# AWehenkel/UMNN

Measured on AMD Instinct MI355X. Metric: umnn_maf_log_density_evals_per_s, higher is better.
Workload: dtype f32 via f16x3-split MFMA (fp32 accumulate)

## Files before the change

### umnn_amd/csrc/cc_api.hip

```cpp
#include <atomic>
#include <cmath>
#include <cstring>
#include <mutex>
#include <unordered_map>
#include <vector>

#include "cc_host.h"

static thread_local char g_err[512] = "";
static thread_local const char* g_last_kernel = "";
static std::atomic<long long> g_launches{0};

int umnn_fail(int code, const char* msg) {
    snprintf(g_err, sizeof(g_err), "%s", msg);
    return code;
}

int umnn_check(hipError_t e, const char* what) {
    if (e == hipSuccess) return 0;
    snprintf(g_err, sizeof(g_err), "%s: %s", what, hipGetErrorString(e));
    return (int)e;
}

static std::atomic<const char*> g_last_of[3] = {{""}, {""}, {""}};
void umnn_note_launch(const char* kernel_name) {
    g_last_kernel = kernel_name;
    const int tag = !strncmp(kernel_name, "cc_bwd_dh", 9) || !strncmp(kernel_name, "cc_bwd_reduce", 13) ? UMNN_PROF_FINISH
                    : !strncmp(kernel_name, "cc_bwd", 6) ? UMNN_PROF_BACKWARD : UMNN_PROF_FORWARD;
    g_last_of[tag].store(kernel_name, std::memory_order_relaxed);
    g_launches.fetch_add(1, std::memory_order_relaxed);
}
static std::atomic<long long> g_made_launches{0};
static std::atomic<const char*> g_last_made{""};
void umnn_note_made_launch(const char* kernel_name) {
    g_last_made.store(kernel_name, std::memory_order_relaxed);
    g_made_launches.fetch_add(1, std::memory_order_relaxed);
}
extern "C" long long umnn_made_launch_count(void) { return g_made_launches.load(std::memory_order_relaxed); }
extern "C" const char* umnn_last_made_kernel_name(void) { return g_last_made.load(std::memory_order_relaxed); }
extern "C" const char* umnn_last_kernel_name_of(int tag) {
    return tag >= 0 && tag <= 2 ? g_last_of[tag].load(std::memory_order_relaxed) : "";
}

int umnn_num_cus() {
    static std::atomic<int> cus[64];
    int dev = 0;
    if (hipGetDevice(&dev) != hipSuccess || dev < 0 || dev >= 64) return 256;
    int v = cus[dev].load(std::memory_order_relaxed);
    if (!v) {
        hipDeviceProp_t prop;
        v = hipGetDeviceProperties(&prop, dev) == hipSuccess && prop.multiProcessorCount > 0 ? prop.multiProcessorCount : 256;
        cus[dev].store(v, std::memory_order_relaxed);
    }
    return v;
}

int umnn_ovf_slot(unsigned long long** flag, unsigned long long* gen) {
    static std::mutex mu;
    static unsigned long long* ring[64] = {nullptr};
    static std::atomic<unsigned long long> next{1};
    int dev = 0;
    if (int rc = umnn_check(hipGetDevice(&dev), "hipGetDevice")) return rc;
// ... 22 lines not shown
int umnn_allow_lds(const void* fn, size_t bytes) {
    struct Key { int dev; const void* fn; bool operator==(const Key& o) const { return dev == o.dev && fn == o.fn; } };
    struct Hash { size_t operator()(const Key& k) const { return std::hash<const void*>()(k.fn) ^ ((size_t)k.dev * 0x9e3779b97f4a7c15ull); } };
    static std::mutex mu;
    static std::unordered_map<Key, size_t, Hash> granted;
    int dev = 0;
    if (int rc = umnn_check(hipGetDevice(&dev), "hipGetDevice")) return rc;
    std::lock_guard<std::mutex> lk(mu);
    auto it = granted.find(Key{dev, fn});
    if (it != granted.end() && it->second >= bytes) return 0;
    if (int rc = umnn_check(hipFuncSetAttribute(fn, hipFuncAttributeMaxDynamicSharedMemorySize, (int)bytes),
                            "hipFuncSetAttribute(MaxDynamicSharedMemorySize)"))
        return rc;
    granted[Key{dev, fn}] = bytes;
    return 0;
}

static int env_int(const char* name, int dflt) { const char* e = getenv(name); return e && *e ? atoi(e) : dflt; }
static void load_env(UmnnOptions& o) {
    int fp = UMNN_PRECISION_F16X3, bp = UMNN_PRECISION_BF16X3;
    if (const char* ev = getenv("UMNN_FWD_PRECISION")) {
        if (!strcmp(ev, "fp32")) fp = UMNN_PRECISION_FP32;
        else if (!strcmp(ev, "bf16x6")) fp = UMNN_PRECISION_BF16X6;
        else if (!strcmp(ev, "bf16x3")) fp = UMNN_PRECISION_BF16X3;
    }
    if (const char* ev = getenv("UMNN_BWD_PRECISION")) bp = !strcmp(ev, "fp32") ? UMNN_PRECISION_FP32 : UMNN_PRECISION_BF16X3;
    o.fwd_precision = fp; o.bwd_precision = bp;
    int v = env_int("UMNN_FWD_P", -1); o.fwd_p = v == 1 || v == 2 ? v : -1;
    v = env_int("UMNN_FWD_NS", -1); o.fwd_ns = v == 1 || v == 2 || v == 4 ? v : -1;
    v = env_int("UMNN_FWD_TAIL", -1); o.fwd_tail = v < 0 ? -1 : (v != 0);
    v = env_int("UMNN_FWD_PIPE", 1); o.fwd_pipe = v >= 0 && v <= 2 ? v : 1;
    o.fwd_pad = env_int("UMNN_FWD_PAD", 1) != 0;
    v = env_int("UMNN_FWD_PAD_MIN", 1); o.fwd_pad_min = v >= 0 && v <= 127 ? v : 1;
    v = env_int("UMNN_BWD_NS", -1); o.bwd_ns = v >= 1 && v <= 32 ? v : -1;
    o.bwd_swp = env_int("UMNN_BWD_SWP", 1) != 0;
    o.bwd_ws = env_int("UMNN_BWD_WS", 1) != 0;
    v = env_int("UMNN_BWD_WS16", 1); o.bwd_ws16 = v >= 0 && v <= 2 ? v : 1;
    v = env_int("UMNN_FRONT_BWD2", 1); o.front_bwd2 = v >= 0 && v <= 2 ? v : 1;
}
UmnnOptions& umnn_options() {
    static UmnnOptions opts;
    static std::once_flag once;
    std::call_once(once, [] { load_env(opts); });
    return opts;
}
extern "C" int umnn_reload_env(void) { load_env(umnn_options()); return 0; }

static std::atomic<int>* option_slot(const char* name) {
    UmnnOptions& o = umnn_options();
    if (!name) return nullptr;
    if (!strcmp(name, "fwd_precision")) return &o.fwd_precision;
    if (!strcmp(name, "bwd_precision")) return &o.bwd_precision;
    if (!strcmp(name, "fwd_p")) return &o.fwd_p;
    if (!strcmp(name, "fwd_ns")) return &o.fwd_ns;
    if (!strcmp(name, "fwd_tail")) return &o.fwd_tail;
    if (!strcmp(name, "fwd_pipe")) return &o.fwd_pipe;
    if (!strcmp(name, "fwd_pad")) return &o.fwd_pad;
    if (!strcmp(name, "fwd_pad_min")) return &o.fwd_pad_min;
    if (!strcmp(name, "bwd_ns")) return &o.bwd_ns;
    if (!strcmp(name, "bwd_swp")) return &o.bwd_swp;
    if (!strcmp(name, "bwd_ws")) return &o.bwd_ws;
    if (!strcmp(name, "bwd_ws16")) return &o.bwd_ws16;
    if (!strcmp(name, "front_bwd2")) return &o.front_bwd2;
    return nullptr;
}
static bool option_value_ok(const char* name, int v) {
    if (!strcmp(name, "fwd_precision")) return v >= UMNN_PRECISION_FP32 && v <= UMNN_PRECISION_F16X3;
    if (!strcmp(name, "bwd_precision")) return v == UMNN_PRECISION_FP32 || v == UMNN_PRECISION_BF16X3;
    if (!strcmp(name, "fwd_p")) return v == -1 || v == 1 || v == 2;
    if (!strcmp(name, "fwd_ns")) return v == -1 || v == 1 || v == 2 || v == 4;
    if (!strcmp(name, "fwd_tail")) return v == -1 || v == 0 || v == 1;
    if (!strcmp(name, "fwd_pipe")) return v >= 0 && v <= 2;
    if (!strcmp(name, "fwd_pad")) return v == 0 || v == 1;
    if (!strcmp(name, "fwd_pad_min")) return v >= 0 && v <= 127;
    if (!strcmp(name, "bwd_ns")) return v == -1 || (v >= 1 && v <= 32);
    if (!strcmp(name, "bwd_swp")) return v == 0 || v == 1;
    if (!strcmp(name, "bwd_ws")) return v == 0 || v == 1;
    if (!strcmp(name, "bwd_ws16")) return v >= 0 && v <= 2;
    if (!strcmp(name, "front_bwd2")) return v >= 0 && v <= 2;
    return true;
}
extern "C" int umnn_set_option(const char* name, int value) {
    std::atomic<int>* s = option_slot(name);
    if (!s) return umnn_fail(UMNN_EINVAL, "umnn_set_option: unknown option name");
    if (!option_value_ok(name, value)) return umnn_fail(UMNN_EINVAL, "umnn_set_option: value out of range for this option");
    s->store(value, std::memory_order_relaxed);
    return 0;
}
extern "C" int umnn_get_option(const char* name, int* value) {
    std::atomic<int>* s = option_slot(name);
    if (!s || !value) return umnn_fail(UMNN_EINVAL, "umnn_get_option: unknown option name or null output");
    *value = s->load(std::memory_order_relaxed);
    return 0;
}
extern "C" int umnn_set_forward_precision(int mode) {
    if (mode < UMNN_PRECISION_FP32 || mode > UMNN_PRECISION_F16X3) return umnn_fail(UMNN_EINVAL, "unknown precision mode");
    umnn_options().fwd_precision = mode;
    return 0;
}
extern "C" int umnn_get_forward_precision(void) { return umnn_options().fwd_precision; }
extern "C" int umnn_set_backward_precision(int mode) {
    if (mode != UMNN_PRECISION_FP32 && mode != UMNN_PRECISION_BF16X3)
        return umnn_fail(UMNN_EINVAL, "backward precision must be UMNN_PRECISION_FP32 or UMNN_PRECISION_BF16X3");
    umnn_options().bwd_precision = mode;
    return 0;
}
extern "C" int umnn_get_backward_precision(void) { return umnn_options().bwd_precision; }
// ... 154 lines not shown
```

### umnn_amd/csrc/cc_common.h

```cpp
#pragma once
#include <hip/hip_runtime.h>

#include "../../include/umnn_cc.h"

typedef float f32x4 __attribute__((ext_vector_type(4)));

#define UMNN_WAVES_PER_BLOCK 4
#define UMNN_BLOCK (64 * UMNN_WAVES_PER_BLOCK)

struct MlpDev {
    const float* W[UMNN_MAX_LINEAR];
    const float* b[UMNN_MAX_LINEAR];
    int width[UMNN_MAX_LINEAR + 1];
    int n_linear;
    int t_out[UMNN_MAX_LINEAR];
    int ks_in[UMNN_MAX_LINEAR];
    int lds_off[UMNN_MAX_LINEAR];
    int t_mfma[UMNN_MAX_LINEAR];
    int tail_off;
    int n_tail;
    int hidden_act;
    int out_act;
};

__device__ __forceinline__ int feat_of(int t, int r, int g) { return 16 * t + 4 * r + g; }
__device__ __forceinline__ int fout_of(int t, int rho) { return 16 * t + 4 * (rho & 3) + (rho >> 2); }

__device__ __forceinline__ f32x4 mfma16(float a, float b, f32x4 c) {
    return __builtin_amdgcn_mfma_f32_16x16x4f32(a, b, c, 0, 0, 0);
}

__device__ __forceinline__ unsigned short f32_to_bf16_rn(float x) {
    const unsigned u = __float_as_uint(x);
    return (unsigned short)((u + 0x7fffu + ((u >> 16) & 1u)) >> 16);
}
__device__ __forceinline__ float io_ld(const float* p, long long i, int bf16) {
    return bf16 ? __uint_as_float((unsigned)reinterpret_cast<const unsigned short*>(p)[i] << 16) : p[i];
}
__device__ __forceinline__ void io_st(float* p, long long i, float v, int bf16) {
    if (bf16) reinterpret_cast<unsigned short*>(p)[i] = f32_to_bf16_rn(v);
    else p[i] = v;
}
struct IoView {
    const float* p;
    int bf16;
    __device__ __forceinline__ float operator[](long long i) const { return io_ld(p, i, bf16); }
    __device__ __forceinline__ IoView operator+(long long o) const {
        return IoView{bf16 ? reinterpret_cast<const float*>(reinterpret_cast<const unsigned short*>(p) + o) : p + o, bf16};
    }
};

template <int NT, int CH>
__device__ __forceinline__ void item_embedding_gemm(const IoView& hb, const float* __restrict__ W0, int H1, int E, int d, int g, int p,
                                                    f32x4 (&c)[NT]) {
    for (int se0 = 0; se0 < (E + 3) / 4; se0 += CH) {
        float hv[CH], A[CH][NT];
#pragma unroll
        for (int q = 0; q < CH; ++q) {
            const int e = 4 * (se0 + q) + g;
// ... 92 lines not shown
```

### umnn_amd/csrc/cc_forward_bf16.hip

```cpp
#ifndef UMNN_ASM_TIED
#define UMNN_ASM_TIED 1
#endif
#include "cc_fwd_plan.h"
using namespace UMNN_FWD_NS;
#ifdef UMNN_FWD_PIECE_F16
#define FWD_KNAME "cc_fwd_f16"
#define FWD_LAUNCH umnn_launch_forward_f16
#else
#define FWD_KNAME "cc_fwd_bf16"
#define FWD_LAUNCH umnn_launch_forward_bf16
#endif

typedef void (*fwd_bf16_kernel_t)(const FwdBf16Args);
struct Bf16Variant { int tmax, nparts, p, exact, nrl, pipe, wpb; fwd_bf16_kernel_t fn; const char* name; };
struct Bf16WideFirst { int t1, nrl, p; fwd_bf16_kernel_t fn; const char* name; };
#define BF16_WIDE_FIRST(T, NR, PP) { T, NR, PP, cc_fwd_bf16_kernel<T, 2, PP, true, NR, false, false, 4>, FWD_KNAME "<T1=" #T ",TREST=4,PARTS=2,P=" #PP ",EXACT=1,LIVE=" #NR ">" }
static const Bf16WideFirst kBf16WideFirst[] = { BF16_WIDE_FIRST(5, 13, 1), BF16_WIDE_FIRST(6, 13, 1), BF16_WIDE_FIRST(7, 13, 1), BF16_WIDE_FIRST(8, 13, 1),
                                                BF16_WIDE_FIRST(5, 0, 1), BF16_WIDE_FIRST(6, 0, 1), BF16_WIDE_FIRST(7, 0, 1), BF16_WIDE_FIRST(8, 0, 1) };
#define BF16_VARIANT(T, NP, PP, EX, NR) { T, NP, PP, EX, NR, 0, 4, cc_fwd_bf16_kernel<T, NP, PP, (EX) != 0, NR>, FWD_KNAME "<T=" #T ",PARTS=" #NP ",P=" #PP ",EXACT=" #EX ",LIVE=" #NR ">" }
#define BF16_PIPE_VARIANT(NP, PP, NR) { 4, NP, PP, 1, NR, 1, 4, cc_fwd_bf16_kernel<4, NP, PP, true, NR, true>, FWD_KNAME "<T=4,PARTS=" #NP ",P=" #PP ",EXACT=1,LIVE=" #NR ",PIPE>" }
#define BF16_VARIANT_W8(T, NR) { T, 2, 1, 1, NR, 0, 8, cc_fwd_bf16_kernel<T, 2, 1, true, NR, false, false, 0, 8>, FWD_KNAME "<T=" #T ",PARTS=2,P=1,EXACT=1,LIVE=" #NR ",WAVES=8>" }
static const Bf16Variant kBf16Variants[] = {
    BF16_PIPE_VARIANT(2, 2, 13), BF16_PIPE_VARIANT(2, 2, 0),
    BF16_VARIANT(4, 2, 1, 1, 13), BF16_VARIANT(4, 2, 2, 1, 13),
    BF16_VARIANT(4, 2, 1, 1, 0), BF16_VARIANT(4, 2, 2, 1, 0),
    BF16_VARIANT(2, 2, 1, 0, 0), BF16_VARIANT(2, 2, 2, 0, 0),
    BF16_VARIANT(4, 2, 1, 0, 0), BF16_VARIANT(4, 2, 2, 0, 0),
#ifndef UMNN_FWD_PIECE_F16
    BF16_VARIANT(4, 3, 1, 1, 13), BF16_VARIANT(4, 3, 2, 1, 13), BF16_VARIANT(4, 3, 1, 1, 0), BF16_VARIANT(4, 3, 2, 1, 0),
    BF16_VARIANT(2, 3, 1, 0, 0), BF16_VARIANT(2, 3, 2, 0, 0), BF16_VARIANT(4, 3, 1, 0, 0), BF16_VARIANT(4, 3, 2, 0, 0),
#endif
    BF16_VARIANT(7, 2, 1, 1, 26), BF16_VARIANT(7, 2, 1, 1, 0),
    BF16_VARIANT(5, 2, 1, 1, 0), BF16_VARIANT(6, 2, 1, 1, 0), BF16_VARIANT(8, 2, 1, 1, 0),
    BF16_VARIANT_W8(7, 26), BF16_VARIANT_W8(7, 0), BF16_VARIANT_W8(5, 0), BF16_VARIANT_W8(6, 0), BF16_VARIANT_W8(8, 0),
    BF16_VARIANT(8, 2, 1, 0, 0), BF16_VARIANT(8, 2, 2, 0, 0),
};

int umnn_launch_forward_p32(FwdArgs& a, const umnn_mlp* net, int nb_steps, hipStream_t stream);

struct FwdOvfPlan { int mode; unsigned long long* flag; unsigned long long gen; };
int umnn_ovf_slot(unsigned long long** flag, unsigned long long* gen);
#ifdef UMNN_FWD_PIECE_F16
int umnn_launch_forward_bf16(FwdArgs& a, const umnn_mlp* net, int nparts, int P, int ns, int nb_steps, hipStream_t stream,
                             const FwdOvfPlan* ovf);
#endif

static int launch_planned(fwd_bf16_kernel_t fn, const char* name, unsigned nblk, size_t lds_bytes, FwdBf16Args& args, FwdArgs& a,
                          const umnn_mlp* net, int P, int ns, int nb_steps, hipStream_t stream, const FwdOvfPlan* ovf, int block) {
    args.f.ovf_mode = ovf ? ovf->mode : 0;
    args.f.ovf_flag = ovf ? ovf->flag : nullptr;
    args.f.ovf_gen = ovf ? ovf->gen : 0;
#ifdef UMNN_FWD_PIECE_F16
    umnn_prof_begin(stream);
    hipLaunchKernelGGL(fn, dim3(nblk), dim3(block), lds_bytes, stream, args);
    const FwdOvfPlan second{2, ovf->flag, ovf->gen};
    int rc = umnn_check(hipGetLastError(), "cc_fwd_f16 launch");
    if (!rc) rc = umnn_launch_forward_bf16(a, net, 2, P, ns, nb_steps, stream, &second);
    if (rc == UMNN_EUNSUPPORTED) rc = umnn_fail(UMNN_EUNSUPPORTED, "cc_fwd_f16: the bf16 build has no kernel for the plan of the fp16 launch");
    umnn_prof_end(stream, umnn_cc_forward_flops_per_integral(net, nb_steps) * (double)a.NI);
    umnn_note_launch(name);
    return rc;
#else
    (void)P; (void)ns;
    if (!ovf) umnn_prof_begin(stream);
    hipLaunchKernelGGL(fn, dim3(nblk), dim3(block), lds_bytes, stream, args);
    if (!ovf) {
        umnn_prof_end(stream, umnn_cc_forward_flops_per_integral(net, nb_steps) * (double)a.NI);
        umnn_note_launch(name);
    }
    return umnn_check(hipGetLastError(), "cc_fwd_bf16 launch");
#endif
}

int FWD_LAUNCH(FwdArgs& a, const umnn_mlp* net, int nparts, int P, int ns, int nb_steps,
                             hipStream_t stream, const FwdOvfPlan* ovf) {
    const int L = a.m.n_linear - 1;
    const UmnnOptions& opt = umnn_options();
#ifdef UMNN_FWD_PIECE_F16
    FwdOvfPlan own{1, nullptr, 0};
    if (int rc = umnn_ovf_slot(&own.flag, &own.gen)) return rc;
    ovf = &own;
    const bool fb = false;
#else
    const bool fb = ovf != nullptr;
#endif
    const bool p_forced = opt.fwd_p > 0 || fb, ns_forced = opt.fwd_ns > 0 || fb;
    int tmax = 0;
    for (int l = 1; l <= L; ++l) tmax = a.m.t_out[l] > tmax ? a.m.t_out[l] : tmax;
    int wide = nparts == 2 ? fwd_uniform_wide(a.m, tmax) : 0;
    if (wide && (P == 1 || !p_forced)) P = 1; else wide = 0;
    if (wide && !ns_forced) {
        const long long tiles16 = (a.NI + 15) / 16, slots = (long long)umnn_num_cus() * 8;
        ns = tiles16 * 4 <= slots ? 4 : tiles16 * 2 <= slots ? 2 : 1;
        if (ns > nb_steps + 1) ns = 1;
    }
    FwdBf16Args args;
    args.f = a;
    FwdLayout lay;
    if (nparts == 2 && (P == 1 || !p_forced) && fwd_plan_wide_first(args, nparts, &lay)) {
        if (!ns_forced) {
            const long long tiles16 = (a.NI + 15) / 16, slots = (long long)umnn_num_cus() * 4 * 2;
            ns = tiles16 * 4 <= slots ? 4 : tiles16 * 2 <= slots ? 2 : 1;
            if (ns > nb_steps + 1) ns = 1;
        }
        const size_t lds_bytes = ((size_t)args.f.m.lds_off[L] + (ns > 1 ? UMNN_WAVES_PER_BLOCK * 3 * 16 : 0)) * sizeof(float);
        const Bf16WideFirst* pick = nullptr;
        for (const Bf16WideFirst& v : kBf16WideFirst) if (v.t1 == lay.T && v.nrl == lay.nrl && v.p == 1) pick = &v;
        if (pick && lds_bytes <= 160 * 1024) {
            if (int rc = umnn_allow_lds((const void*)pick->fn, lds_bytes)) return rc;
            args.f.ns = ns;
            args.f.ngroups = (unsigned)((a.NI + 16 * pick->p - 1) / (16 * pick->p));
            const unsigned gpb = UMNN_WAVES_PER_BLOCK / ns;
            const unsigned nblk = (args.f.ngroups + gpb - 1) / gpb;
            return launch_planned(pick->fn, pick->name, nblk, lds_bytes, args, a, net, pick->p, ns, nb_steps, stream, ovf, UMNN_BLOCK);
        }
        args.f = a;
    }
    if (a.z2_save) return UMNN_EUNSUPPORTED;
    lay = fwd_plan_images(args, nparts, tmax, wide, nparts == 2 && opt.fwd_pad, opt.fwd_pad_min);
    const int T = lay.T, exact = lay.exact, nrl = lay.nrl;
    const bool want_pipe = opt.fwd_pipe != 0 && L >= 2;
#ifndef UMNN_FWD_PIECE_F16
    if (opt.fwd_pipe == 2 && !fb && exact && T == 4 && nparts == 2 && nrl == 13) {
        const int rc = umnn_launch_forward_p32(a, net, nb_steps, stream);
        if (rc != UMNN_EUNSUPPORTED) return rc;
    }
#endif
    if (want_pipe && exact && T == 4 && nparts == 2 && !p_forced && !ns_forced &&
        (a.NI + 15) / 16 >= 2LL * umnn_num_cus() * 4) { P = 2; ns = 1; }
    int wpb = wide && exact && 2 * ((size_t)args.f.m.lds_off[L] * sizeof(float) + 1024) > 160 * 1024 ? 8 : UMNN_WAVES_PER_BLOCK;
    size_t lds_bytes = ((size_t)args.f.m.lds_off[L] + (ns > 1 ? wpb * 3 * P * 16 : 0)) * sizeof(float);
    if (lds_bytes > 160 * 1024 && wpb == 8) { wpb = UMNN_WAVES_PER_BLOCK; lds_bytes = ((size_t)args.f.m.lds_off[L] + (ns > 1 ? wpb * 3 * P * 16 : 0)) * sizeof(float); }
    if (lds_bytes > 160 * 1024) return UMNN_EUNSUPPORTED;
    const Bf16Variant* pick = nullptr;
    for (int ex = exact; ex >= 0 && !pick; --ex)
        for (int pass = 0; pass < 2 && !pick; ++pass)
            for (const Bf16Variant& v : kBf16Variants)
                if (v.tmax == T && v.nparts == nparts && v.p == P && v.exact == ex && (!v.pipe || want_pipe) && v.wpb == (ex ? wpb : 4) &&
                    (pass == 0 ? (ex && nrl && v.nrl == nrl) : v.nrl == 0)) { pick = &v; break; }
    if (!pick) return UMNN_EUNSUPPORTED;
    fwd_bf16_kernel_t kfn = pick->fn;
    const char* kname = pick->name;
    if (int rc = umnn_allow_lds((const void*)kfn, lds_bytes)) return rc;
    args.f.ns = ns;
    args.f.ngroups = (unsigned)((a.NI + 16 * P - 1) / (16 * P));
    const unsigned gpb = pick->wpb / ns;
    const unsigned nblk = (args.f.ngroups + gpb - 1) / gpb;
    return launch_planned(kfn, kname, nblk, lds_bytes, args, a, net, P, ns, nb_steps, stream, ovf, 64 * pick->wpb);
}
```

### umnn_amd/csrc/cc_fwd_bf16_kernel.h

```cpp
#pragma once
#include <type_traits>
#include <utility>
#include "cc_bf16.h"
#include "cc_fwd_shared.h"
#include "cc_host.h"

#ifdef UMNN_FWD_PIECE_F16
#define UMNN_FWD_NS fwd_f16
#else
#define UMNN_FWD_NS fwd_bf16
#endif
namespace UMNN_FWD_NS {
#ifdef UMNN_FWD_PIECE_F16
typedef _Float16 pc_x8 __attribute__((ext_vector_type(8)));
typedef _Float16 pc_x4 __attribute__((ext_vector_type(4)));
typedef _Float16 pc_x2 __attribute__((ext_vector_type(2)));
constexpr unsigned PC_MINUS_ONE = 0xBC00u;
constexpr bool PC_F16 = true;
__device__ __forceinline__ f32x4 pc_mfma(u32x4 a, u32x4 b, f32x4 c) {
    return __builtin_amdgcn_mfma_f32_16x16x32_f16(__builtin_bit_cast(pc_x8, a), __builtin_bit_cast(pc_x8, b), c, 0, 0, 0);
}
__device__ __forceinline__ f32x4 pc_mfma_k16(u32x2 a, u32x2 b, f32x4 c) {
    return __builtin_amdgcn_mfma_f32_16x16x16f16(__builtin_bit_cast(pc_x4, a), __builtin_bit_cast(pc_x4, b), c, 0, 0, 0);
}
// ... 20 lines not shown
}
#ifdef UMNN_FWD_PIECE_F16
__device__ __forceinline__ unsigned pc_lo_pair(float x0, float x1, unsigned hi) {
    unsigned lo = __float_as_uint(x0);
    asm("v_fma_mixlo_f16 %0, %1, -1.0, %0 op_sel_hi:[1,0,0]" : "+v"(lo) : "v"(hi));
    asm("v_fma_mixhi_f16 %0, %1, -1.0, %2 op_sel:[1,0,0] op_sel_hi:[1,0,0]" : "+v"(lo) : "v"(hi), "v"(x1));
    return lo;
}
template <int I>
__device__ __forceinline__ void pc_sub_halves(f32x4& v, unsigned bits) {
    float x0 = v[I], x1 = v[I + 1];
    asm("v_fma_mix_f32 %0, %1, -1.0, %0 op_sel_hi:[1,0,0]" : "+v"(x0) : "v"(bits));
    asm("v_fma_mix_f32 %0, %1, -1.0, %0 op_sel:[1,0,0] op_sel_hi:[1,0,0]" : "+v"(x1) : "v"(bits));
    v[I] = x0; v[I + 1] = x1;
}
#endif
template <int NPARTS>
__device__ __forceinline__ void pc_split_pair(float x0, float x1, unsigned (&out)[NPARTS]) {
#ifdef UMNN_FWD_PIECE_F16
    if constexpr (NPARTS == 2) {
        out[0] = pc_cvt_pk(x0, x1);
        out[1] = pc_lo_pair(x0, x1, out[0]);
        return;
    }
#endif
#pragma unroll
    for (int k = 0; k < NPARTS; ++k) {
        const unsigned bits = pc_cvt_pk(x0, x1);
        out[k] = bits;
        if (k + 1 < NPARTS) { x0 -= pc_lo_f32(bits); x1 -= pc_hi_f32(bits); }
    }
}

template <int NPARTS, int MERGE_FROM = 0>
__device__ __forceinline__ void stage_bf16_images(const MlpDev& m, const int* ks32, const int* off16, const int* half_in,
                                                  unsigned short* lds16, int tid, int nthreads) {
    const int L = m.n_linear - 1;
    for (int l = 1; l < L; ++l) {
        const int Hin = m.width[l], Hout = m.width[l + 1];
        const int ks = ks32[l], to = m.t_out[l + 1];
        const float* __restrict__ W = m.W[l];
        const float* __restrict__ b = m.b[l];
        unsigned short* img = lds16 + off16[l];
        auto wv = [&](int fo, int fi) {
            float v = 0.f;
            if (fo < Hout) {
                if (fi < Hin) v = W[fo * Hin + fi];
                else if (fi == Hin) v = b[fo];
            } else if (fo == Hout && fi == Hin) {
                v = 1.f;
            }
            return v;
        };
        auto split8 = [&](const float (&v)[8], unsigned (&pk)[NPARTS][4]) {
#pragma unroll
            for (int e = 0; e < 4; ++e) {
                unsigned q[NPARTS];
                pc_split_pair<NPARTS>(v[2 * e], v[2 * e + 1], q);
#pragma unroll
                for (int part = 0; part < NPARTS; ++part) pk[part][e] = q[part];
            }
        };
        const int total = to * ks * 64;
        for (int idx = tid; idx < total; idx += nthreads) {
            const int ln = idx & 63, ts = idx >> 6;
            const int s = ts % ks, t = ts / ks;
// ... 25 lines not shown
                unsigned q0[NPARTS], q1[NPARTS];
                pc_split_pair<NPARTS>(wv(fo, feat_of(2 * ks, 0, g)), wv(fo, feat_of(2 * ks, 1, g)), q0);
                pc_split_pair<NPARTS>(wv(fo, feat_of(2 * ks, 2, g)), wv(fo, feat_of(2 * ks, 3, g)), q1);
#pragma unroll
                for (int part = 0; part < NPARTS; ++part)
                    *reinterpret_cast<u32x2*>(himg + (t * NPARTS + part) * 256 + ln * 4) = u32x2{q0[part], q1[part]};
            }
        }
    }
}

struct Bf16Plan {
    int ks32[UMNN_MAX_LINEAR];
    int off16[UMNN_MAX_LINEAR];
    int half_in[UMNN_MAX_LINEAR];
    int scratch_off_floats;
};

struct SolveArgs {
    long long t_stride = 0, x_stride = 0;
    const float* scale_row = nullptr;
    const float* off_row = nullptr;
    int off_h0 = 0;
    int* status = nullptr;
    float lo = 0.f, hi = 0.f, tol = 0.f;
    int block = 0;
};
constexpr int SOLVE_CLAMPED = 1 << 16, SOLVE_CAPPED = 1 << 17, SOLVE_NONFINITE = 1 << 18;

struct FwdBf16Args {
    FwdArgs f;
    Bf16Plan pl;
    SolveArgs sv;
};

template <int... I, class F>
__device__ __forceinline__ void static_for(std::integer_sequence<int, I...>, F&& f) {
    (f(std::integral_constant<int, I>{}), ...);
}
template <int TMAX, int NPARTS, int P, bool EXACT, int NRL, bool PIPE = false, int INV = 0, int TREST = 0, int WPB = UMNN_WAVES_PER_BLOCK>
__global__ __launch_bounds__(64 * WPB) void cc_fwd_bf16_kernel(const FwdBf16Args args) {
    static_assert(TREST == 0 || (EXACT && !PIPE && TREST < TMAX && (TREST & 1) == 0), "wide-first-layer variants: exact, plain loop");
    static_assert(!INV || (P == 1 && !PIPE), "inversion variants: plain loop, one tile per wave");
    constexpr int KSM = TMAX / 2;
    constexpr int NLIVE = (NRL > 0 && TREST == 0) ? NRL : 4 * TMAX;
    constexpr int NREST = TREST > 0 ? (NRL > 0 ? NRL : 4 * TREST) : NLIVE;
    constexpr bool MERGE = EXACT && TMAX == 4 && NRL == 13 && NPARTS == 2 && TREST == 0;
    constexpr bool MERGE_REST = EXACT && TREST == 4 && NRL == 13 && NPARTS == 2;
    extern __shared__ __attribute__((aligned(16))) float lds[];
    const FwdArgs& a = args.f;
    const MlpDev& m = a.m;
    const int tid = threadIdx.x, lane = tid & 63;
    const int wid = __builtin_amdgcn_readfirstlane(tid >> 6);
    const int g = lane >> 4, p = lane & 15;
    const int L = m.n_linear - 1;
    const int H1 = m.width[1], HL = m.width[L];
    const int E = a.E, d = a.d, n = a.n;
    const float slope = m.hidden_act == UMNN_ACT_RELU ? 0.f : 0.01f;
    unsigned short* lds16 = reinterpret_cast<unsigned short*>(lds);
    if (a.ovf_mode == 2 && *a.ovf_flag < a.ovf_gen) return;

    stage_bf16_images<NPARTS, MERGE ? 1 : MERGE_REST ? 2 : 0>(m, args.pl.ks32, args.pl.off16, args.pl.half_in, lds16, tid, 64 * WPB);
    __syncthreads();

    const int ns = a.ns;
    const int sub = wid / ns, part = wid % ns;
    const unsigned gpb = WPB / ns;
    const unsigned grp = xcd_remap(blockIdx.x, gridDim.x) * gpb + sub;
    bool live = grp < a.ngroups;
    if (a.ovf_mode == 2 && live) {
        if constexpr (INV == 2) {
            long long q = (long long)grp * 16 + p;
            if (q >= a.NI) q = a.NI - 1;
            const float v = a.inv_x[q * args.sv.x_stride + a.inv_j];
            live = __any(v != v);
        } else if constexpr (INV) { const float v = a.inv_x[(long long)grp * d + a.inv_j]; live = v != v; }
        else live = fwd_group_marked<P>(a, grp, p);
    }
    const int k_lo = (int)(((long long)part * (n + 1)) / ns);
    const int k_hi = (int)(((long long)(part + 1) * (n + 1)) / ns);

    float Facc[P], fxv[P], fx0v[P], xv[P], x0v[P], dxv[P];
    bool ok[P];
    long long qv[P];
#pragma unroll
    for (int pt = 0; pt < P; ++pt) { Facc[pt] = 0.f; fxv[pt] = 0.f; fx0v[pt] = 0.f; ok[pt] = false; qv[pt] = 0; dxv[pt] = 0.f; }

    if (live) {
        IoView hb[P];
        int sv_col = a.inv_j;
#pragma unroll
        for (int pt = 0; pt < P; ++pt) {
            if constexpr (INV == 2) {
                const long long q = (long long)grp * 16 + p;
                ok[pt] = q < a.NI;
                qv[pt] = ok[pt] ? q : a.NI - 1;
                xv[pt] = 0.f; x0v[pt] = 0.f; dxv[pt] = 0.f;
                long long bi = qv[pt];
                if (args.sv.block) { bi = qv[pt] / d; sv_col = (int)(qv[pt] - bi * d); }
                hb[pt] = IoView{a.h, a.h_bf16} + (bi * ((long long)E * d) + sv_col);
            } else if constexpr (INV) {
// ... 78 lines not shown
            for (int pt = 0; pt < 2; ++pt)
#pragma unroll
                for (int ks = 0; ks < 2; ++ks)
#pragma unroll
                    for (int k2 = 0; k2 < 2; ++k2) bf[pt][ks][k2] = u32x4{0u, 0u, 0u, 0u};
            u32x4 sel[2];
            {
                const unsigned rho = lane & 15, slot = rho & 3;
                const unsigned v = ((unsigned)(lane >> 4) == (rho >> 2)) ? (PC_MINUS_ONE << (16 * (slot & 1))) : 0u;
                sel[0] = u32x4{slot < 2 ? v : 0u, slot < 2 ? 0u : v, 0u, 0u};
                sel[1] = u32x4{0u, 0u, slot < 2 ? v : 0u, slot < 2 ? 0u : v};
            }
            float rem_a = 0.f;
            unsigned rem_hi = 0u;
            auto frag = [&](int l, int t, int ks, int k2) {
                return *reinterpret_cast<const u32x4*>(lds16 + (l - 1) * (16 * 512) + lane * 8 + ((t * 2 + ks) * 2 + k2) * 512);
            };
#pragma unroll
            for (int t = 0; t < 4; ++t)
#pragma unroll
                for (int ks = 0; ks < 2; ++ks)
#pragma unroll
                    for (int k2 = 0; k2 < 2; ++k2) wf[t][ks][k2] = frag(1, t, ks, k2);
            auto mfma_slot = [&](auto ic, const u32x4 (&bfin)[2][2], f32x4 (&acc)[4]) {
                constexpr int i = decltype(ic)::value;
                constexpr int t = i % 4;
                constexpr int ks = MERGE ? (i / 4 >= 3) : i / 12;
                constexpr int term = MERGE ? (i / 4) % 3 : (i / 4) % 3;
                constexpr int wa = (MERGE && ks == 1) ? i / 4 - 3 : (term == 2 ? 1 : 0);
                constexpr int ba = (MERGE && ks == 1) ? i / 4 - 3 : (term == 1 ? 1 : 0);
                if constexpr (i < 4) acc[t] = pc_mfma(wf[t][ks][wa], bfin[ks][ba], f32x4{0.f, 0.f, 0.f, 0.f});
                else acc[t] = pc_mfma(wf[t][ks][wa], bfin[ks][ba], acc[t]);
            };
            auto reload_slot = [&](auto ic, int lnext) {
                constexpr int i = decltype(ic)::value;
                if constexpr (MERGE) {
                    constexpr int step = i / 4, t = i % 4;
                    if constexpr (step >= 1) wf[t][step >= 3][(step - 1) & 1] = frag(lnext, t, step >= 3, (step - 1) & 1);
                } else {
                    constexpr int ks = i / 12, term = (i / 4) % 3, t = i % 4;
                    if constexpr (term == 1) wf[t][ks][0] = frag(lnext, t, ks, 0);
                    if constexpr (term == 2) wf[t][ks][1] = frag(lnext, t, ks, 1);
                }
            };
            auto pack_slot = [&](auto ic, auto first, f32x4 (&z)[4], u32x4 (&bfout)[2][2], float tkv, const f32x4 (&cv)[TMAX]) {
                constexpr int i = decltype(ic)::value;
                constexpr int MODE = decltype(first)::value;
                constexpr bool FIRST = MODE == 1, PRE = MODE == 2;
                constexpr int t_act = MERGE ? (i <= 3 ? 0 : (i >= 4 && i <= 7) ? 1 : (i >= 12 && i <= 15) ? 2 : -1)
                                            : (i <= 3 ? 0 : (i >= 4 && i <= 7) ? 1 : (i >= 10 && i <= 13) ? 2 : (i >= 14 && i <= 17) ? 3 : -1);
                constexpr int r_act = MERGE ? (t_act == 0 ? i : t_act == 1 ? i - 4 : i - 12)
                                            : (t_act == 0 ? i : t_act == 1 ? i - 4 : t_act == 2 ? i - 10 : i - 14);
                constexpr int t_hi = MERGE ? (i == 16 ? 2 : -1) : -1;
                constexpr int t_lo = MERGE ? (i == 17 ? 0 : i == 18 ? 1 : i == 19 ? 2 : -1) : (i >= 20 ? i - 20 : -1);
                constexpr int T3A = MERGE ? 10 : -1, T3B = MERGE ? 11 : -1;
                constexpr int QCVT = (!MERGE && i == 18) ? 1 : (i == 8 ? 0 : -1);
                constexpr int QSEL = (!MERGE && i == 19) ? 1 : (i == 9 ? 0 : -1);
                if constexpr (t_act >= 0 && !PRE) {
                    if constexpr (FIRST) z[t_act][r_act] = fmaf(w1x[t_act][r_act], tkv, cv[t_act][r_act]);
                    z[t_act][r_act] = hidden_act_f(z[t_act][r_act], slope);
                }
                if constexpr (QCVT >= 0) {
                    constexpr int ta = 2 * QCVT, tb = 2 * QCVT + 1;
                    const unsigned a0 = pc_cvt_pk(z[ta][0], z[ta][1]);
                    const unsigned a1 = pc_cvt_pk(z[ta][2], z[ta][3]);
                    const unsigned b0 = pc_cvt_pk(z[tb][0], z[tb][1]);
                    const unsigned b1 = pc_cvt_pk(z[tb][2], z[tb][3]);
                    bfout[QCVT][0] = u32x4{a0, a1,
                                           b0, b1};
                }
#ifdef UMNN_FWD_PIECE_F16
// ... 388 lines not shown
            }
            const float span = br_right - br_left;
            const float lo = __fadd_rn(__fmul_rn((float)((double)(m > 0 ? m - 1 : 0) / 9.0), span), br_left);
            const float hi = __fadd_rn(__fmul_rn((float)((double)(m < 9 ? m + 1 : 9) / 9.0), span), br_left);
            br_best = __fadd_rn(__fmul_rn((float)((double)m / 9.0), span), br_left);
            const bool below = zm < inv_target;
            br_left = below ? br_best : lo;
            br_right = below ? hi : br_best;
        }
        }
        if constexpr (INV == 2) {
            const bool defer = a.ovf_mode == 1 && sv_bad;
            if (sv_mine && g == 0 && part == 0) {
                if (!sv_done) sv_stat |= SOLVE_CAPPED;
                if (sv_bad) sv_stat |= SOLVE_NONFINITE;
                a.inv_x[qv[0] * args.sv.x_stride + a.inv_j] = sv_bad ? __builtin_nanf("") : sv_x;
                if (!defer) {
                    if (a.fx) a.fx[qv[0]] = sv_fx;
                    if (args.sv.status) args.sv.status[qv[0]] = sv_stat;
                }
            }
            if (__any(defer) && lane == 0 && part == 0) atomicMax(a.ovf_flag, a.ovf_gen);
        }
        if constexpr (INV == 1) {
            const bool defer = a.ovf_mode == 1 && __any(inv_bad);
            if (ok[0] && lane == 0 && part == 0) {
                a.inv_x[qv[0] * d + a.inv_j] = (defer || inv_nan) ? __builtin_nanf("") : br_best;
                if (defer) atomicMax(a.ovf_flag, a.ovf_gen);
            }
        }
        }
    }
    if constexpr (!INV) fwd_epilogue<P>(a, lds, Facc, fxv, fx0v, ok, qv, dxv, live, part, ns, wid, g, p);
}

}
```

### umnn_amd/csrc/cc_fwd_plan.h

```cpp
#pragma once
#include "cc_fwd_bf16_kernel.h"

namespace UMNN_FWD_NS {

struct FwdLayout { int T, exact, nrl, wide; };

inline int fwd_tile_bucket(int tmax) { return tmax <= 2 ? 2 : tmax <= 4 ? 4 : 8; }

inline int fwd_uniform_wide(const MlpDev& m, int tmax) {
    int wide = tmax >= 5 ? tmax : 0;
    for (int l = 1; l < m.n_linear && wide; ++l) if (m.t_out[l] != wide) wide = 0;
    return wide;
}

inline void fwd_close_images(FwdBf16Args& args, int off16) { args.f.m.lds_off[args.f.m.n_linear - 1] = (((off16 + 1) / 2) + 3) & ~3; }

inline bool fwd_plan_wide_first(FwdBf16Args& args, int nparts, FwdLayout* lay) {
    MlpDev& m = args.f.m;
    const int L = m.n_linear - 1, T1 = m.t_out[1];
    if (L < 2 || T1 < 5 || T1 > 8) return false;
    for (int l = 2; l <= L; ++l) if (m.t_out[l] > 4) return false;
    int off16 = 0;
    for (int l = 1; l <= L; ++l) {
        args.pl.ks32[l] = l == 1 ? T1 / 2 : 2;
// ... 8 lines not shown
    int nrest = m.ks_in[2];
    for (int l = 2; l <= L; ++l) if (m.ks_in[l] != nrest) nrest = 0;
    *lay = FwdLayout{T1, 1, nrest == 13 ? 13 : 0, 0};
    return true;
}

inline FwdLayout fwd_plan_images(FwdBf16Args& args, int nparts, int tmax, int wide, bool pad, int pad_min) {
    MlpDev& m = args.f.m;
    const int L = m.n_linear - 1;
    FwdLayout lay{wide ? wide : fwd_tile_bucket(tmax), 1, m.ks_in[1], wide};
    int off16 = 0;
    for (int l = 1; l <= L; ++l) {
        args.pl.half_in[l] = wide ? (wide & 1) : 0;
        args.pl.ks32[l] = wide ? wide / 2 : (m.t_out[l] + 1) / 2;
    }
    for (int l = 1; l < L; ++l) {
        args.pl.off16[l] = off16;
        off16 += m.t_out[l + 1] * (args.pl.ks32[l] * nparts * 512 + args.pl.half_in[l] * nparts * 256);
    }
    for (int l = 1; l <= L; ++l) {
        lay.exact = lay.exact && m.t_out[l] == lay.T;
        if (m.ks_in[l] != lay.nrl) lay.nrl = 0;
    }
    if (pad && !lay.exact && !wide && tmax <= 4 && tmax >= pad_min) {
        lay.T = 4; lay.exact = 1; lay.nrl = 0;
        for (int l = 1; l <= L; ++l) { m.t_out[l] = 4; args.pl.ks32[l] = 2; }
        off16 = 0;
        for (int l = 1; l < L; ++l) { args.pl.off16[l] = off16; off16 += 4 * 2 * nparts * 512; }
    }
    fwd_close_images(args, off16);
    return lay;
}

}
```

### umnn_amd/csrc/cc_host.h

```cpp
#pragma once
#include <atomic>
#include <cstdio>
#include <cstdlib>

#include "cc_common.h"

int umnn_fail(int code, const char* msg);
int umnn_check(hipError_t e, const char* what);
int umnn_prepare_mlp(const umnn_mlp* net, int E, MlpDev* out, int* tmax, int* ksu);
int umnn_check_io(const umnn_io* io);
int umnn_num_cus();

struct UmnnOptions {
    std::atomic<int> fwd_precision{UMNN_PRECISION_F16X3};
    std::atomic<int> bwd_precision{UMNN_PRECISION_BF16X3};
    std::atomic<int> fwd_p{-1};
    std::atomic<int> fwd_ns{-1};
    std::atomic<int> fwd_tail{-1};
    std::atomic<int> fwd_pipe{1};
    std::atomic<int> fwd_pad{1};
    std::atomic<int> fwd_pad_min{1};
    std::atomic<int> bwd_ns{-1};
    std::atomic<int> bwd_ws{1};
    std::atomic<int> bwd_ws16{1};
    std::atomic<int> front_bwd2{1};
    std::atomic<int> bwd_swp{1};
};
UmnnOptions& umnn_options();
int umnn_allow_lds(const void* fn, size_t bytes);
void umnn_note_launch(const char* kernel_name);
void umnn_note_made_launch(const char* kernel_name);
long long umnn_param_count(const umnn_mlp* net);

void umnn_prof_begin(hipStream_t stream);
void umnn_prof_end(hipStream_t stream, double flops, int tag = UMNN_PROF_FORWARD);
```

Before: 633,000.

## Add persistent-grid mode to pipelined forward kernel and skip dead tile-3 reloads

The pipelined forward kernel gains an outer loop over virtual blocks, so the grid can be capped at the number of resident workgroups (queried through the occupancy API and cached per device). Each workgroup then walks through several virtual blocks instead of launching one block per group. In the merged pipeline, reloads of weight fragments for tile-3 rows that are beyond the live output rows are skipped. A host check verifies those rows are zero in the weight images. The persistent loop saves repeated block launch and LDS weight staging, but it adds loop overhead and opaque lane-index barriers that may hurt scheduling.

```diff
diff --git a/umnn_amd/csrc/cc_api.hip b/umnn_amd/csrc/cc_api.hip
--- a/umnn_amd/csrc/cc_api.hip
+++ b/umnn_amd/csrc/cc_api.hip
@@ -23,11 +23,11 @@
 }
 
 static std::atomic<const char*> g_last_of[3] = {{""}, {""}, {""}};
-void umnn_note_launch(const char* kernel_name) {
+void umnn_note_launch(const char* kernel_name, const char* plan_name) {
     g_last_kernel = kernel_name;
     const int tag = !strncmp(kernel_name, "cc_bwd_dh", 9) || !strncmp(kernel_name, "cc_bwd_reduce", 13) ? UMNN_PROF_FINISH
                     : !strncmp(kernel_name, "cc_bwd", 6) ? UMNN_PROF_BACKWARD : UMNN_PROF_FORWARD;
-    g_last_of[tag].store(kernel_name, std::memory_order_relaxed);
+    g_last_of[tag].store(plan_name ? plan_name : kernel_name, std::memory_order_relaxed);
     g_launches.fetch_add(1, std::memory_order_relaxed);
 }
 static std::atomic<long long> g_made_launches{0};
@@ -116,6 +116,8 @@
     v = env_int("UMNN_FWD_PIPE", 1); o.fwd_pipe = v >= 0 && v <= 2 ? v : 1;
     o.fwd_pad = env_int("UMNN_FWD_PAD", 1) != 0;
     v = env_int("UMNN_FWD_PAD_MIN", 1); o.fwd_pad_min = v >= 0 && v <= 127 ? v : 1;
+    o.fwd_persist = env_int("UMNN_FWD_PERSIST", 1) != 0;
+    v = env_int("UMNN_FWD_PERSIST_WGS", 0); o.fwd_persist_wgs = v >= 0 && v <= 65536 ? v : 0;
     v = env_int("UMNN_BWD_NS", -1); o.bwd_ns = v >= 1 && v <= 32 ? v : -1;
     o.bwd_swp = env_int("UMNN_BWD_SWP", 1) != 0;
     o.bwd_ws = env_int("UMNN_BWD_WS", 1) != 0;
@@ -141,6 +143,8 @@
     if (!strcmp(name, "fwd_pipe")) return &o.fwd_pipe;
     if (!strcmp(name, "fwd_pad")) return &o.fwd_pad;
     if (!strcmp(name, "fwd_pad_min")) return &o.fwd_pad_min;
+    if (!strcmp(name, "fwd_persist")) return &o.fwd_persist;
+    if (!strcmp(name, "fwd_persist_wgs")) return &o.fwd_persist_wgs;
     if (!strcmp(name, "bwd_ns")) return &o.bwd_ns;
     if (!strcmp(name, "bwd_swp")) return &o.bwd_swp;
     if (!strcmp(name, "bwd_ws")) return &o.bwd_ws;
@@ -157,6 +161,8 @@
     if (!strcmp(name, "fwd_pipe")) return v >= 0 && v <= 2;
     if (!strcmp(name, "fwd_pad")) return v == 0 || v == 1;
     if (!strcmp(name, "fwd_pad_min")) return v >= 0 && v <= 127;
+    if (!strcmp(name, "fwd_persist")) return v == 0 || v == 1;
+    if (!strcmp(name, "fwd_persist_wgs")) return v >= 0 && v <= 65536;
     if (!strcmp(name, "bwd_ns")) return v == -1 || (v >= 1 && v <= 32);
     if (!strcmp(name, "bwd_swp")) return v == 0 || v == 1;
     if (!strcmp(name, "bwd_ws")) return v == 0 || v == 1;
diff --git a/umnn_amd/csrc/cc_common.h b/umnn_amd/csrc/cc_common.h
--- a/umnn_amd/csrc/cc_common.h
+++ b/umnn_amd/csrc/cc_common.h
@@ -23,8 +23,8 @@
     int out_act;
 };
 
-__device__ __forceinline__ int feat_of(int t, int r, int g) { return 16 * t + 4 * r + g; }
-__device__ __forceinline__ int fout_of(int t, int rho) { return 16 * t + 4 * (rho & 3) + (rho >> 2); }
+__host__ __device__ __forceinline__ int feat_of(int t, int r, int g) { return 16 * t + 4 * r + g; }
+__host__ __device__ __forceinline__ int fout_of(int t, int rho) { return 16 * t + 4 * (rho & 3) + (rho >> 2); }
 
 __device__ __forceinline__ f32x4 mfma16(float a, float b, f32x4 c) {
     return __builtin_amdgcn_mfma_f32_16x16x4f32(a, b, c, 0, 0, 0);
diff --git a/umnn_amd/csrc/cc_forward_bf16.hip b/umnn_amd/csrc/cc_forward_bf16.hip
--- a/umnn_amd/csrc/cc_forward_bf16.hip
+++ b/umnn_amd/csrc/cc_forward_bf16.hip
@@ -1,6 +1,8 @@
 #ifndef UMNN_ASM_TIED
 #define UMNN_ASM_TIED 1
 #endif
+#include <map>
+#include <mutex>
 #include "cc_fwd_plan.h"
 using namespace UMNN_FWD_NS;
 #ifdef UMNN_FWD_PIECE_F16
@@ -12,14 +14,15 @@
 #endif
 
 typedef void (*fwd_bf16_kernel_t)(const FwdBf16Args);
-struct Bf16Variant { int tmax, nparts, p, exact, nrl, pipe, wpb; fwd_bf16_kernel_t fn; const char* name; };
+struct Bf16Variant { int tmax, nparts, p, exact, nrl, pipe, wpb; fwd_bf16_kernel_t fn; const char* name; const char* pname; };
 struct Bf16WideFirst { int t1, nrl, p; fwd_bf16_kernel_t fn; const char* name; };
 #define BF16_WIDE_FIRST(T, NR, PP) { T, NR, PP, cc_fwd_bf16_kernel<T, 2, PP, true, NR, false, false, 4>, FWD_KNAME "<T1=" #T ",TREST=4,PARTS=2,P=" #PP ",EXACT=1,LIVE=" #NR ">" }
 static const Bf16WideFirst kBf16WideFirst[] = { BF16_WIDE_FIRST(5, 13, 1), BF16_WIDE_FIRST(6, 13, 1), BF16_WIDE_FIRST(7, 13, 1), BF16_WIDE_FIRST(8, 13, 1),
                                                 BF16_WIDE_FIRST(5, 0, 1), BF16_WIDE_FIRST(6, 0, 1), BF16_WIDE_FIRST(7, 0, 1), BF16_WIDE_FIRST(8, 0, 1) };
-#define BF16_VARIANT(T, NP, PP, EX, NR) { T, NP, PP, EX, NR, 0, 4, cc_fwd_bf16_kernel<T, NP, PP, (EX) != 0, NR>, FWD_KNAME "<T=" #T ",PARTS=" #NP ",P=" #PP ",EXACT=" #EX ",LIVE=" #NR ">" }
-#define BF16_PIPE_VARIANT(NP, PP, NR) { 4, NP, PP, 1, NR, 1, 4, cc_fwd_bf16_kernel<4, NP, PP, true, NR, true>, FWD_KNAME "<T=4,PARTS=" #NP ",P=" #PP ",EXACT=1,LIVE=" #NR ",PIPE>" }
-#define BF16_VARIANT_W8(T, NR) { T, 2, 1, 1, NR, 0, 8, cc_fwd_bf16_kernel<T, 2, 1, true, NR, false, false, 0, 8>, FWD_KNAME "<T=" #T ",PARTS=2,P=1,EXACT=1,LIVE=" #NR ",WAVES=8>" }
+#define BF16_VARIANT(T, NP, PP, EX, NR) { T, NP, PP, EX, NR, 0, 4, cc_fwd_bf16_kernel<T, NP, PP, (EX) != 0, NR>, FWD_KNAME "<T=" #T ",PARTS=" #NP ",P=" #PP ",EXACT=" #EX ",LIVE=" #NR ">", nullptr }
+#define BF16_PIPE_VARIANT(NP, PP, NR) { 4, NP, PP, 1, NR, 1, 4, cc_fwd_bf16_kernel<4, NP, PP, true, NR, true>, FWD_KNAME "<T=4,PARTS=" #NP ",P=" #PP ",EXACT=1,LIVE=" #NR ",PIPE>", \
+                                        FWD_KNAME "<T=4,PARTS=" #NP ",P=" #PP ",EXACT=1,LIVE=" #NR ",PIPE,PERSIST>" }
+#define BF16_VARIANT_W8(T, NR) { T, 2, 1, 1, NR, 0, 8, cc_fwd_bf16_kernel<T, 2, 1, true, NR, false, false, 0, 8>, FWD_KNAME "<T=" #T ",PARTS=2,P=1,EXACT=1,LIVE=" #NR ",WAVES=8>", nullptr }
 static const Bf16Variant kBf16Variants[] = {
     BF16_PIPE_VARIANT(2, 2, 13), BF16_PIPE_VARIANT(2, 2, 0),
     BF16_VARIANT(4, 2, 1, 1, 13), BF16_VARIANT(4, 2, 2, 1, 13),
@@ -45,28 +48,54 @@
                              const FwdOvfPlan* ovf);
 #endif
 
-static int launch_planned(fwd_bf16_kernel_t fn, const char* name, unsigned nblk, size_t lds_bytes, FwdBf16Args& args, FwdArgs& a,
+static unsigned fwd_persistent_grid(const Bf16Variant& v, unsigned nblk, size_t lds_bytes, int ns, int block) {
+    const UmnnOptions& opt = umnn_options();
+    if (!v.pipe || !v.pname || ns != 1 || !opt.fwd_persist) return nblk;
+    struct Key { int dev; const void* fn; size_t lds; bool operator<(const Key& o) const { return dev != o.dev ? dev < o.dev : fn != o.fn ? fn < o.fn : lds < o.lds; } };
+    static std::mutex mu;
+    static std::map<Key, int> cache;
+    int dev = 0, occ = 0;
+    if (hipGetDevice(&dev) != hipSuccess) return nblk;
+    {
+        std::lock_guard<std::mutex> lk(mu);
+        const Key key{dev, (const void*)v.fn, lds_bytes};
+        auto it = cache.find(key);
+        if (it == cache.end()) {
+            if (hipOccupancyMaxActiveBlocksPerMultiprocessor(&occ, (const void*)v.fn, block, lds_bytes) != hipSuccess || occ < 1) occ = 0;
+            it = cache.emplace(key, occ).first;
+        }
+        occ = it->second;
+    }
+    if (occ < 1) return nblk;
+    unsigned long long resident = (unsigned long long)occ * (unsigned)umnn_num_cus();
+    const int cap = opt.fwd_persist_wgs;
+    if (cap > 0 && (unsigned long long)cap < resident) resident = (unsigned)cap;
+    return nblk > resident ? (unsigned)resident : nblk;
+}
+
+static int launch_planned(fwd_bf16_kernel_t fn, const char* name, const char* plan_name, unsigned nblk, unsigned grid, size_t lds_bytes, FwdBf16Args& args, FwdArgs& a,
                           const umnn_mlp* net, int P, int ns, int nb_steps, hipStream_t stream, const FwdOvfPlan* ovf, int block) {
     args.f.ovf_mode = ovf ? ovf->mode : 0;
     args.f.ovf_flag = ovf ? ovf->flag : nullptr;
     args.f.ovf_gen = ovf ? ovf->gen : 0;
+    args.vblk = nblk;
 #ifdef UMNN_FWD_PIECE_F16
     umnn_prof_begin(stream);
-    hipLaunchKernelGGL(fn, dim3(nblk), dim3(block), lds_bytes, stream, args);
+    hipLaunchKernelGGL(fn, dim3(grid), dim3(block), lds_bytes, stream, args);
     const FwdOvfPlan second{2, ovf->flag, ovf->gen};
     int rc = umnn_check(hipGetLastError(), "cc_fwd_f16 launch");
     if (!rc) rc = umnn_launch_forward_bf16(a, net, 2, P, ns, nb_steps, stream, &second);
     if (rc == UMNN_EUNSUPPORTED) rc = umnn_fail(UMNN_EUNSUPPORTED, "cc_fwd_f16: the bf16 build has no kernel for the plan of the fp16 launch");
     umnn_prof_end(stream, umnn_cc_forward_flops_per_integral(net, nb_steps) * (double)a.NI);
-    umnn_note_launch(name);
+    umnn_note_launch(name, plan_name);
     return rc;
 #else
     (void)P; (void)ns;
     if (!ovf) umnn_prof_begin(stream);
-    hipLaunchKernelGGL(fn, dim3(nblk), dim3(block), lds_bytes, stream, args);
+    hipLaunchKernelGGL(fn, dim3(grid), dim3(block), lds_bytes, stream, args);
     if (!ovf) {
         umnn_prof_end(stream, umnn_cc_forward_flops_per_integral(net, nb_steps) * (double)a.NI);
-        umnn_note_launch(name);
+        umnn_note_launch(name, plan_name);
     }
     return umnn_check(hipGetLastError(), "cc_fwd_bf16 launch");
 #endif
@@ -112,7 +141,7 @@
             args.f.ngroups = (unsigned)((a.NI + 16 * pick->p - 1) / (16 * pick->p));
             const unsigned gpb = UMNN_WAVES_PER_BLOCK / ns;
             const unsigned nblk = (args.f.ngroups + gpb - 1) / gpb;
-            return launch_planned(pick->fn, pick->name, nblk, lds_bytes, args, a, net, pick->p, ns, nb_steps, stream, ovf, UMNN_BLOCK);
+            return launch_planned(pick->fn, pick->name, nullptr, nblk, nblk, lds_bytes, args, a, net, pick->p, ns, nb_steps, stream, ovf, UMNN_BLOCK);
         }
         args.f = a;
     }
@@ -146,5 +175,9 @@
     args.f.ngroups = (unsigned)((a.NI + 16 * P - 1) / (16 * P));
     const unsigned gpb = pick->wpb / ns;
     const unsigned nblk = (args.f.ngroups + gpb - 1) / gpb;
-    return launch_planned(kfn, kname, nblk, lds_bytes, args, a, net, P, ns, nb_steps, stream, ovf, 64 * pick->wpb);
+    const unsigned grid = fwd_persistent_grid(*pick, nblk, lds_bytes, ns, 64 * pick->wpb);
+    const char* plan_name = grid < nblk ? pick->pname : nullptr;
+    if (!fwd_tile3_dead_rows_zero(args.f.m, pick->pipe ? pick->nrl : 0))
+        return umnn_fail(UMNN_EINVAL, "cc_fwd: a row of output tile 3 that the pipelined loop does not reload is not zero in the weight images");
+    return launch_planned(kfn, kname, plan_name, nblk, grid, lds_bytes, args, a, net, P, ns, nb_steps, stream, ovf, 64 * pick->wpb);
 }
diff --git a/umnn_amd/csrc/cc_fwd_bf16_kernel.h b/umnn_amd/csrc/cc_fwd_bf16_kernel.h
--- a/umnn_amd/csrc/cc_fwd_bf16_kernel.h
+++ b/umnn_amd/csrc/cc_fwd_bf16_kernel.h
@@ -76,6 +76,10 @@
     }
 }
 
+__host__ __device__ __forceinline__ int fwd_image_src(int Hin, int Hout, int fo, int fi) {
+    if (fo < Hout) return fi < Hin ? 1 : fi == Hin ? 2 : 0;
+    return fo == Hout && fi == Hin ? 3 : 0;
+}
 template <int NPARTS, int MERGE_FROM = 0>
 __device__ __forceinline__ void stage_bf16_images(const MlpDev& m, const int* ks32, const int* off16, const int* half_in,
                                                   unsigned short* lds16, int tid, int nthreads) {
@@ -167,8 +171,10 @@
     FwdArgs f;
     Bf16Plan pl;
     SolveArgs sv;
+    unsigned vblk = 0;
 };
 
+__device__ __forceinline__ int opaque_lane_index(int v) { asm volatile("" : "+v"(v)); return v; }
 template <int... I, class F>
 __device__ __forceinline__ void static_for(std::integer_sequence<int, I...>, F&& f) {
     (f(std::integral_constant<int, I>{}), ...);
@@ -187,7 +193,7 @@
     const MlpDev& m = a.m;
     const int tid = threadIdx.x, lane = tid & 63;
     const int wid = __builtin_amdgcn_readfirstlane(tid >> 6);
-    const int g = lane >> 4, p = lane & 15;
+    const int g0 = lane >> 4, p0 = lane & 15;
     const int L = m.n_linear - 1;
     const int H1 = m.width[1], HL = m.width[L];
     const int E = a.E, d = a.d, n = a.n;
@@ -201,7 +207,11 @@
     const int ns = a.ns;
     const int sub = wid / ns, part = wid % ns;
     const unsigned gpb = WPB / ns;
-    const unsigned grp = xcd_remap(blockIdx.x, gridDim.x) * gpb + sub;
+    unsigned vb = blockIdx.x;
+    const unsigned nvb = PIPE ? args.vblk : gridDim.x;
+    for (;;) {
+    const int g = PIPE ? opaque_lane_index(g0) : g0, p = PIPE ? opaque_lane_index(p0) : p0;
+    const unsigned grp = xcd_remap(vb, nvb) * gpb + sub;
     bool live = grp < a.ngroups;
     if (a.ovf_mode == 2 && live) {
         if constexpr (INV == 2) {
@@ -346,11 +356,14 @@
                 if constexpr (i < 4) acc[t] = pc_mfma(wf[t][ks][wa], bfin[ks][ba], f32x4{0.f, 0.f, 0.f, 0.f});
                 else acc[t] = pc_mfma(wf[t][ks][wa], bfin[ks][ba], acc[t]);
             };
+            const bool live3 = fout_of(3, lane & 15) < 4 * NLIVE;
             auto reload_slot = [&](auto ic, int lnext) {
                 constexpr int i = decltype(ic)::value;
                 if constexpr (MERGE) {
                     constexpr int step = i / 4, t = i % 4;
-                    if constexpr (step >= 1) wf[t][step >= 3][(step - 1) & 1] = frag(lnext, t, step >= 3, (step - 1) & 1);
+                    if constexpr (step >= 1 && t == 3) {
+                        if (live3) wf[3][step >= 3][(step - 1) & 1] = frag(lnext, 3, step >= 3, (step - 1) & 1);
+                    } else if constexpr (step >= 1) wf[t][step >= 3][(step - 1) & 1] = frag(lnext, t, step >= 3, (step - 1) & 1);
                 } else {
                     constexpr int ks = i / 12, term = (i / 4) % 3, t = i % 4;
                     if constexpr (term == 1) wf[t][ks][0] = frag(lnext, t, ks, 0);
@@ -805,6 +818,10 @@
         }
     }
     if constexpr (!INV) fwd_epilogue<P>(a, lds, Facc, fxv, fx0v, ok, qv, dxv, live, part, ns, wid, g, p);
-}
-
-}
+    if constexpr (!PIPE) break;
+    vb += gridDim.x;
+    if (vb >= nvb) break;
+    }
+}
+
+}
diff --git a/umnn_amd/csrc/cc_fwd_plan.h b/umnn_amd/csrc/cc_fwd_plan.h
--- a/umnn_amd/csrc/cc_fwd_plan.h
+++ b/umnn_amd/csrc/cc_fwd_plan.h
@@ -64,4 +64,16 @@
     return lay;
 }
 
+inline bool fwd_tile3_dead_rows_zero(const MlpDev& m, int nrl_pipe) {
+    if (nrl_pipe != 13) return true;
+    for (int l = 1; l + 1 < m.n_linear; ++l)
+        for (int rho = 0; rho < 16; ++rho) {
+            const int fo = fout_of(3, rho);
+            if (fo < 4 * nrl_pipe) continue;
+            for (int fi = 0; fi < 16 * 4; ++fi)
+                if (fwd_image_src(m.width[l], m.width[l + 1], fo, fi) != 0) return false;
+        }
+    return true;
 }
+
+}
diff --git a/umnn_amd/csrc/cc_host.h b/umnn_amd/csrc/cc_host.h
--- a/umnn_amd/csrc/cc_host.h
+++ b/umnn_amd/csrc/cc_host.h
@@ -20,6 +20,8 @@
     std::atomic<int> fwd_pipe{1};
     std::atomic<int> fwd_pad{1};
     std::atomic<int> fwd_pad_min{1};
+    std::atomic<int> fwd_persist{1};
+    std::atomic<int> fwd_persist_wgs{0};
     std::atomic<int> bwd_ns{-1};
     std::atomic<int> bwd_ws{1};
     std::atomic<int> bwd_ws16{1};
@@ -28,7 +30,7 @@
 };
 UmnnOptions& umnn_options();
 int umnn_allow_lds(const void* fn, size_t bytes);
-void umnn_note_launch(const char* kernel_name);
+void umnn_note_launch(const char* kernel_name, const char* plan_name = nullptr);
 void umnn_note_made_launch(const char* kernel_name);
 long long umnn_param_count(const umnn_mlp* net);
 
```

Measured after the change: 606,700. 0.958x the previous value.
